# PatrykChrabaszcz/HpBandSter

Measured on AMD Instinct MI355X. Metric: candidate KDE evals/sec (cand×obs pairs) at D=32, 1/2/4/8 MI355X; % VALU peak, higher is better.
Workload: dtype f16 MFMA coarse pre-screen (1 product per dim, rigorous bound), f32 accumulate, f64 re-score

## Files before the change

hpbandster_amd/csrc/hbx_acq_impl.h:

```cpp
#pragma once
#include "hbx_kde_impl.h"
#include "hbx_score.h"

__device__ __forceinline__ void est_interval(const KdeEst e, float* lo, float* hi, float* pt) {
  const float m = fmaxf(e.lpos, e.lneg);
  if (m == -INFINITY) {
    *lo = *hi = *pt = -INFINITY;
    return;
  }
  const float a = __expf(e.lpos - m), b = __expf(e.lneg - m);
  const float S = a - b, E = e.err * (a + b) + 1e-6f * (a + b);
  *pt = S > 0.f ? m + __logf(S) : -INFINITY;
  *hi = (S + E) > 0.f ? m + __logf(S + E) + 1e-6f * fabsf(m) + 1e-5f : -INFINITY;
  *lo = (S - E) > 0.f ? m + __logf(S - E) - 1e-6f * fabsf(m) - 1e-5f : -INFINITY;
}

struct ScoreIv {
  float slo, shi, lpt, gpt;
  bool lnan, of, one;
};
__device__ __forceinline__ ScoreIv score_interval(const KdeEst a, const KdeEst b, const ScoreFloor F) {
  const float C = F.C;
  ScoreIv v;
  v.of = false;
// ... 30 lines not shown
}

#define HBX_EST_NOT_EVAL (-3.f)
__device__ __forceinline__ ScoreIv score_interval_l_only(const KdeEst a, const ScoreFloor F) {
  const float C = F.C;
  ScoreIv v;
  v.of = false;
  v.one = false;
  v.gpt = NAN;
  v.lnan = a.lpos != a.lpos;
  if (v.lnan) {
    v.slo = v.shi = NAN;
    v.lpt = NAN;
    return v;
  }
  float llo, lhi;
  est_interval(a, &llo, &lhi, &v.lpt);
  v.of = lhi > 700.f;
  v.slo = C - fmaxf(lhi, C) - F.w;
  v.shi = INFINITY;
  return v;
}

__device__ __forceinline__ KdeEst merge_splits(const KdeEst* __restrict__ e, int64_t stride, int64_t i, int nsplit) {
  KdeEst p[OBS_SPLIT_MAX];
#pragma unroll
  for (int r = 0; r < OBS_SPLIT_MAX; ++r) p[r] = r < nsplit ? e[(int64_t)r * stride + i] : kde_est_neutral();
  auto lae = [](float x, float y) {
    const float m = fmaxf(x, y);
    return m == -INFINITY ? m : m + __logf(__expf(x - m) + __expf(y - m));
  };
  KdeEst a = p[0];
#pragma unroll
  for (int r = 1; r < OBS_SPLIT_MAX; ++r) {
    if (r < nsplit) {
      const KdeEst b = p[r];
      if (a.lpos != a.lpos || b.lpos != b.lpos) {
        a.lpos = NAN;
      } else {
        a.lpos = lae(a.lpos, b.lpos);
        a.lneg = lae(a.lneg, b.lneg);
        const float ml = fmaxf(a.lpos > -INFINITY ? fabsf(a.lpos) : 0.f, a.lneg > -INFINITY ? fabsf(a.lneg) : 0.f);
        a.err = fmaxf(a.err, b.err) + 0x1p-18f + ml * 0x1p-22f;
      }
    }
  }
  return a;
}

__device__ __forceinline__ double bohb_score(double g, double l, double f) {
  return ((g > f) ? g : f) / ((f > l) ? f : l);
}

__device__ __forceinline__ double exact_rel(const KdeParams* __restrict__ P, const KdeEst e) {
  const double base = (8.0 * (double)P->D + 160.0) * 0x1p-52;
  if (!P->has_neg) return base;
  if (e.err < -1.5f) return INFINITY;
  const float m = fmaxf(e.lpos, e.lneg);
  if (!(m > -INFINITY)) return base;
  const float a = __expf(e.lpos - m), b = __expf(e.lneg - m);
  const float den = fabsf(a - b) - (e.err + 1e-6f) * (a + b);
  if (!(den > 0.f)) return INFINITY;
  return base * (double)((a + b) / den) * 1.01;
}

__device__ __forceinline__ double score_rel(const KdeParams* __restrict__ Pg, const KdeParams* __restrict__ Pb,
                                            const KdeEst* __restrict__ el, const KdeEst* __restrict__ eg,
                                            int64_t i) {
  return exact_rel(Pg, el[i]) + exact_rel(Pb, eg[i]) + 0x1p-51;
}
// ... 5 lines not shown
```

hpbandster_amd/csrc/hbx_acquire.h:

```cpp
#pragma once
#include "hbx_score.h"

struct KdePairRef {
  int32_t D;
  const void* params_good;
  const float* table_good;
  const double* X_good;
  const int64_t* rows_good;
  int32_t variant_good;
  const void* params_bad;
  const float* table_bad;
  const double* X_bad;
  const int64_t* rows_bad;
  int32_t variant_bad, dc_pad, du_pad;
  int64_t nmax;
  ScoreFloor floor;
  const KdeParams* Pg() const { return (const KdeParams*)params_good; }
  const KdeParams* Pb() const { return (const KdeParams*)params_bad; }
};

struct WsLayout {
  size_t res, U, count, flags, segcnt, segnear, best, key, first1, rescue, est_l, est_g, lo, list, near, exact_l,
      exact_g, part, total;
  size_t stage, seeds, surv, lpart, bmax;
// ... 55 lines not shown
int acq_check(const char* who, const KdePairRef& p, const double* cand, int64_t Nc, const void* workspace);
int acq_plan(const KdePairRef& p, bool fast, AcqPlan* plan);
int acq_score(const AcqPlan& plan, const KdePairRef& p, const AcqWs& a, const ScoreRequest& rq, int64_t batch_B,
              ScoreResult* out);
#ifndef HBX_STAGED_MIN_PAIRS
#define HBX_STAGED_MIN_PAIRS 1e9
#endif
#ifndef HBX_STAGED_TOPK_MIN_PAIRS
#define HBX_STAGED_TOPK_MIN_PAIRS 4e9
#endif
bool acq_staged_supported(const AcqPlan& plan);
int acq_score_staged(const AcqPlan& plan, const KdePairRef& p, const double* cand, int64_t Nc, const AcqWs& a,
                     hipEvent_t* ev, hipStream_t s, bool tail);
int staged_score_l(const AcqPlan& plan, const KdePairRef& p, const double* cand, int64_t Nc, const AcqWs& a,
                   hipEvent_t* ev, hipStream_t s, uint32_t* lkey, uint32_t* hist, int32_t hist_words,
                   unsigned* lhi_blocks = nullptr);
int staged_score_seeds(const AcqPlan& plan, const KdePairRef& p, const double* cand, int64_t Nc, const AcqWs& a,
                       hipStream_t s, bool mark_rest, bool update_u, unsigned lhi_blocks = 0);
int staged_score_survivors(const AcqPlan& plan, const KdePairRef& p, const double* cand, int64_t Nc, const AcqWs& a,
                           hipStream_t s, bool lonly);
int acq_exact_only_init(int64_t Nc, uint32_t seg, const AcqWs& a, hipStream_t s);
#define EXACT_SCAN_MAX 1024
int acq_exact(const KdePairRef& p, const double* cand, int64_t Nc, const AcqWs& a, bool scan, bool combine,
              hipStream_t s);
```

hpbandster_amd/csrc/hbx_common.h:

```cpp
#pragma once

#include <hip/hip_runtime.h>
#include <stdint.h>
#include <stdlib.h>

#define HBX_MAX_D 256
#define HBX_LO_TERMS 32
#define HBX_WAVE 64

#include "hbx.h"

int hbx_fail(int code, const char* fmt, ...);

#define HBX_HIP(call)                                                                 \
  do {                                                                                \
    hipError_t _e = (call);                                                           \
    if (_e != hipSuccess)                                                             \
      return hbx_fail(HBX_ERR_HIP, "%s failed: %s (%s:%d)", #call, hipGetErrorString(_e), \
                      __FILE__, __LINE__);                                            \
  } while (0)

#define HBX_LAUNCH_CHECK()                                                            \
  do {                                                                                \
    hipError_t _e = hipGetLastError();                                                \
// ... 15 lines not shown
static inline bool hbx_staged_tail() { return hbx_switch_on("HBX_STAGED_TAIL"); }
static inline bool hbx_stage1_lhi() { return hbx_switch_on("HBX_STAGE1_LHI"); }

struct KdeParams {
  int32_t n;
  int32_t D;
  int32_t dc;
  int32_t du;
  int32_t nconst;
  int32_t nan_all;
  int32_t has_neg;
  int32_t unsupported;
  int32_t stride;
  int32_t dc_pad;
  int32_t du_pad;
  int32_t exact_only;
  double log_norm;
  double m0_log2;
  double lb_sum;
  double prod_bw_c;
  float cmax;
  float sum_abs_delta;
  float cmax2;
  int32_t pad1;
  int32_t kc;
  int32_t hmode;
  int32_t nsc;
  int32_t chunk_floats;
  int32_t oh_total;
  int32_t coarse_off;
  int32_t coarse_chunk_floats;
  const double* X;
  const int64_t* rows;
  int32_t oh_dim[64];
  int32_t oh_level[64];
  int32_t oh_col[64];
  double oh_val[64];
  int32_t oh_start[64];
  int32_t cat_maxcode[HBX_MAX_D];
  int32_t cont_dim[HBX_MAX_D];
  double cont_scale[HBX_MAX_D];
  double center[HBX_MAX_D];
  float xmax[HBX_MAX_D];
  int32_t cat_dim[HBX_MAX_D];
  float cat_delta[HBX_MAX_D];
  float cat_negf[HBX_MAX_D];
  int32_t const_dim[HBX_MAX_D];
// ... 73 lines not shown
```

hpbandster_amd/csrc/hbx_exact.hip:

```cpp
#include "hbx_acquire.h"
#include "hbx_exact_impl.h"

#ifndef EXACT_ACQ_THREADS
#define EXACT_ACQ_THREADS 256
#endif
struct ExactScan {
  const float* lo;
  int64_t Nc;
  const uint32_t* U;
  const int32_t* flags;
  const int32_t* first1;
  int32_t* list;
  int32_t* count;
  int32_t* rescue_cnt;
};
template <bool SCAN>
__global__ __launch_bounds__(EXACT_ACQ_THREADS) void kde_exact_kernel(
    const double* __restrict__ cand, int32_t D,
    const KdeParams* __restrict__ Pg, const double* __restrict__ Xg, const int64_t* __restrict__ rows_g,
    const KdeParams* __restrict__ Pb, const double* __restrict__ Xb, const int64_t* __restrict__ rows_b,
    const int32_t* __restrict__ list_in, const int32_t* __restrict__ count, int32_t nbuf, double* __restrict__ part,
    double* __restrict__ exact_l, double* __restrict__ exact_g, ExactScan sc) {
  __shared__ ExactShared sh;
  __shared__ int32_t slist[SCAN ? EXACT_SCAN_MAX : 1];
  __shared__ int32_t swc[EXACT_ACQ_THREADS / 64];
  int cnt;
  const int32_t* list = list_in;
  if constexpr (SCAN) {
    const float u = hbx_ord2f(sc.U[0]);
    const bool all = (sc.flags[0] & 1) != 0;
    const int32_t f1 = sc.first1[0];
    const int lane = threadIdx.x & 63, wv = threadIdx.x >> 6;
    int base = 0;
    for (int64_t c0 = 0; c0 < sc.Nc; c0 += EXACT_ACQ_THREADS) {
      const int64_t i = c0 + threadIdx.x;
      bool in = false;
      if (i < sc.Nc) {
        const float l = sc.lo[i];
        in = (l == l && (all || l <= u)) || (int32_t)i == f1;
      }
      const uint64_t b = __ballot(in);
      if (lane == 0) swc[wv] = __popcll(b);
      __syncthreads();
      int off = base, tot = 0;
#pragma unroll
      for (int w = 0; w < EXACT_ACQ_THREADS / 64; ++w) {
        off += w < wv ? swc[w] : 0;
        tot += swc[w];
      }
      if (in) slist[off + __popcll(b & ((1ull << lane) - 1))] = (int32_t)i;
      base += tot;
      __syncthreads();
    }
    cnt = base;
    list = slist;
    if (blockIdx.x == 0) {
      for (int k = threadIdx.x; k < cnt; k += EXACT_ACQ_THREADS) sc.list[k] = slist[k];
      if (threadIdx.x == 0) {
        *sc.count = cnt;
        if (sc.rescue_cnt) *sc.rescue_cnt = 0;
      }
    }
  } else {
    cnt = *count;
  }
  const bool split = cnt <= EXACT_SPLIT_CAP;
  const int per = split ? nbuf * PW_SPLIT_UNITS : 1;
  const int64_t items = (int64_t)cnt * 2 * per;
  for (int64_t item = blockIdx.x; item < items; item += gridDim.x) {
    const int64_t pk = item / per;
    const int p = (int)(pk >> 1);
    const bool isl = pk & 1;
    const KdeParams* P = isl ? Pg : Pb;
    const double* X = isl ? Xg : Xb;
    const int64_t* rows = isl ? rows_g : rows_b;
    if (split) {
      const int r = (int)(item % per), b = r / PW_SPLIT_UNITS, u = r % PW_SPLIT_UNITS;
      const int n = P->n, c = b * PW_BUF;
      if (c >= n) continue;
      const int m = (n - c) < PW_BUF ? (n - c) : PW_BUF;
      int off, len;
      if (!pw_unit<PW_SPLIT_CUT>(m, u, &off, &len)) continue;
      exact_setup(P, D, cand + (int64_t)list[p] * D, &sh);
      const double v = exact_unit<PW_SPLIT_LEVELS>(X, D, rows, P, c + off, len, &sh);
      if (threadIdx.x == 0) part[pk * per + r] = v;
    } else {
      exact_setup(P, D, cand + (int64_t)list[p] * D, &sh);
      const double v = exact_pdf(X, D, rows, P, &sh);
      if (threadIdx.x == 0) (isl ? exact_l : exact_g)[p] = v;
    }
    __syncthreads();
  }
}

__global__ __launch_bounds__(256) void kde_exact_combine_kernel(const KdeParams* __restrict__ Pg,
                                                                const KdeParams* __restrict__ Pb,
                                                                const int32_t* __restrict__ count, int32_t nbuf,
                                                                const double* __restrict__ part,
                                                                double* __restrict__ exact_l,
                                                                double* __restrict__ exact_g) {
  const int cnt = *count;
  if (cnt > EXACT_SPLIT_CAP) return;
  const int64_t pk = (int64_t)blockIdx.x * 4 + (threadIdx.x >> 6);
  if (pk >= 2 * (int64_t)cnt) return;
  const bool isl = pk & 1;
  const int n = (isl ? Pg : Pb)->n;
  const double* us = part + pk * nbuf * PW_SPLIT_UNITS;
// ... 91 lines not shown
    if ((threadIdx.x & 63) == 0) {
      rm[threadIdx.x >> 6] = m;
      rs[threadIdx.x >> 6] = sm;
    }
    __syncthreads();
    if (threadIdx.x == 0) {
      double M = -INFINITY, Sx = 0.0;
      bool nan = false;
      for (int w = 0; w < 4; ++w) {
        if (rm[w] != rm[w]) nan = true;
        else if (rm[w] > -INFINITY) {
          const double mm = fmax(M, rm[w]);
          Sx = (M > -INFINITY ? Sx * exp(M - mm) : 0.0) + rs[w] * exp(rm[w] - mm);
          M = mm;
        }
      }
      out[p] = (nan || P->has_neg || P->nan_all || P->nconst) ? NAN : (M > -INFINITY ? M + log(Sx) + lconst : -INFINITY);
    }
    __syncthreads();
  }
}

int acq_exact(const KdePairRef& p, const double* cand, int64_t Nc, const AcqWs& a, bool scan, bool combine,
              hipStream_t s) {
  const int nbuf = (int)((p.nmax + PW_BUF - 1) / PW_BUF);
  const ExactScan esc = scan ? ExactScan{a.lo, Nc, a.U, a.flags, a.first1, a.list, a.count, a.rescue} : ExactScan{};
  auto ek = scan ? kde_exact_kernel<true> : kde_exact_kernel<false>;
  hipLaunchKernelGGL(ek, dim3(EXACT_GRID), dim3(EXACT_ACQ_THREADS), 0, s, cand, p.D, p.Pg(), p.X_good, p.rows_good,
                     p.Pb(), p.X_bad, p.rows_bad, a.list, a.count, nbuf, a.part, a.exact_l, a.exact_g, esc);
  HBX_LAUNCH_CHECK();
  if (combine) {
    hipLaunchKernelGGL(kde_exact_combine_kernel, dim3((2 * EXACT_SPLIT_CAP + 3) / 4), dim3(256), 0, s, p.Pg(), p.Pb(),
                       a.count, nbuf, a.part, a.exact_l, a.exact_g);
    HBX_LAUNCH_CHECK();
  }
  return HBX_OK;
}

int hbx_logpdf_exact_listed(const double* cand, int64_t Nc, int32_t D, const KdeParams* P, const double* X,
                            const int64_t* rows, double* out, const int32_t* list, const int32_t* count,
                            bool per_point, hipStream_t s) {
  const unsigned grid = (unsigned)(Nc < EXACT_GRID ? Nc : EXACT_GRID);
  if (per_point) {
    hipLaunchKernelGGL(kde_logpdf_exact_kernel, dim3(grid), dim3(256), 0, s, cand, Nc, D, P, X, rows, out, list, count);
    HBX_LAUNCH_CHECK();
  }
  hipLaunchKernelGGL(kde_pdf_exact_kernel, dim3(grid), dim3(EXACT_THREADS), 0, s, cand, Nc, D, P, X, rows, out, list,
                     count, 1);
  HBX_LAUNCH_CHECK();
  return HBX_OK;
}

// ... 45 lines not shown
```

hpbandster_amd/csrc/hbx_exact_impl.h:

```cpp
#pragma once
#include "hbx_kde_impl.h"
#include "hbx_npexp.h"
#include "hbx_pairwise.h"

struct ExactShared {
  double dens[PW_UNIT_MAX];
  double nsum[PW_LEVELS][128];
  double usum[PW_UNITS];
  double c0[HBX_MAX_D], c1[HBX_MAX_D], xd[HBX_MAX_D];
  int32_t cont[HBX_MAX_D];
};

template <typename PV>
__device__ void exact_setup(const PV* __restrict__ P, int32_t D, const double* __restrict__ x, ExactShared* sh) {
  for (int d = threadIdx.x; d < D; d += blockDim.x) {
    const double h = P->bw[d];
    const bool c = P->vartype[d] == 0;
    sh->cont[d] = c;
    sh->c0[d] = c ? (h * h) * 2. : 1. - h;
    sh->c1[d] = c ? 0. : h / (double)(P->nlev[d] - 1);
    sh->xd[d] = x[d];
  }
  __syncthreads();
}
// ... 3 lines not shown
                             const PV* __restrict__ P, int first, int len, ExactShared* sh) {
  const double pbc = P->prod_bw_c;
  for (int j = threadIdx.x; j < len; j += blockDim.x) {
    const double* xr = X + rows[first + j] * (int64_t)D;
    double p = 1.0;
#pragma unroll 8
    for (int d = 0; d < D; ++d) {
      const double v = xr[d], xv = sh->xd[d];
      double k;
      if (sh->cont[d]) {
        const double diff = v - xv;
        k = HBX_INV_SQRT_2PI * hbx_npexp::exp(-(diff * diff) / sh->c0[d]);
      } else {
        k = (v == xv) ? sh->c0[d] : sh->c1[d];
      }
      p = (d == 0) ? k : p * k;
    }
    sh->dens[j] = p / pbc;
  }
  __syncthreads();
  return np_pairwise_block<LEVELS>(sh->dens, len, sh->nsum);
}

template <typename PV>
__device__ double exact_pdf(const double* __restrict__ X, int32_t D, const int64_t* __restrict__ rows,
                            const PV* __restrict__ P, ExactShared* sh) {
  const int n = P->n;
  double acc = 0.0;
  for (int c = 0; c < n; c += PW_BUF) {
    const int m = (n - c) < PW_BUF ? (n - c) : PW_BUF;
    for (int u = 0; u < PW_UNITS; ++u) {
      int off, len;
      if (!pw_unit(m, u, &off, &len)) continue;
      const double v = exact_unit(X, D, rows, P, c + off, len, sh);
      if (threadIdx.x == 0) sh->usum[u] = v;
    }
    __syncthreads();
    if (threadIdx.x == 0) acc = acc + pw_combine_units(m, sh->usum);
  }
  return acc / (double)n;
}
```

hpbandster_amd/csrc/hbx_kde.hip:

```cpp
#include "hbx_acquire.h"

#include <string.h>

#include <new>

#include "hbx_acq_impl.h"
#include "hbx_host.h"
#include "hbx_pairwise.h"
#include "hbx_rescue_impl.h"


__global__ void acq_init_kernel(uint32_t* U, int32_t* count, int32_t* flags, int32_t* first1, AcqResult* res) {
  if (threadIdx.x == 0 && blockIdx.x == 0) acq_init_state(U, count, flags, first1, res);
}

__global__ void acq_init_batch_kernel(int64_t B, uint32_t* __restrict__ U, int32_t* __restrict__ flags,
                                      int32_t* __restrict__ segcnt, uint64_t* __restrict__ best,
                                      uint64_t* __restrict__ key, int32_t* __restrict__ first1,
                                      int32_t* __restrict__ count, int32_t* __restrict__ segnear) {
  const int64_t b = (int64_t)blockIdx.x * blockDim.x + threadIdx.x;
  if (b == 0) *count = 0;
  if (b < B) {
    U[b] = hbx_f2ord(INFINITY);
    flags[b] = 0;
// ... 580 lines not shown
  const dim3 grid((unsigned)((Nc + 255) / 256));
  bool fuse_combine = false;
  if (Nc > 0) {
    if (plan.exact_only) {
      rc = acq_exact_only_init(Nc, sg, a, s);
      if (rc) return rc;
    } else if (!tail) {
      const CombineRescue rs{cand, p.D, p.Pg(), p.Pb(), a.rescue};
      const bool sgn = KdeVariant::decode(p.variant_good).has_neg;
      const combine_fn cf = !rescue_inline ? kde_combine_kernel<false, false>
                            : sgn          ? kde_combine_kernel<true, true>
                                           : kde_combine_kernel<false, true>;
      hipLaunchKernelGGL(cf, dim3((unsigned)((Nc + 256 * COMBINE_SUB - 1) / (256 * COMBINE_SUB))), dim3(256), 0, s,
                         a.el, a.eg, Nc, sg, logl_out, logg_out, a.lo, a.U, a.flags, a.first1, rs, p.floor);
      HBX_LAUNCH_CHECK();
    }
    const bool scan = !batch_res && Nc <= EXACT_SCAN_MAX && !tail;
    if (!scan && !tail) {
      hipLaunchKernelGGL(kde_shortlist_kernel, grid, dim3(256), 0, s, a.lo, Nc, sg, a.U, a.flags, a.list, a.count,
                         batch_res ? a.segcnt : (int32_t*)nullptr, a.first1, a.rescue);
      HBX_LAUNCH_CHECK();
    }
    fuse_combine = !batch_res && !(plan.exact_only && (logl_out || logg_out));
    rc = acq_exact(p, cand, Nc, a, scan, !fuse_combine, s);
    if (rc) return rc;
    if (plan.exact_only && (logl_out || logg_out)) {
      hipLaunchKernelGGL(kde_exact_logs_kernel, grid, dim3(256), 0, s, a.list, a.count, a.exact_l, a.exact_g, logl_out,
                         logg_out);
      HBX_LAUNCH_CHECK();
    }
  }
  if (!batch_res) {
    hipLaunchKernelGGL(kde_final_kernel, dim3(1), dim3(256), 0, s, a.list, a.count, a.exact_l, a.exact_g, a.flags,
                       c.index_base, p.Pg(), p.Pb(), a.el, a.eg, a.near, a.res,
                       (int32_t)((p.nmax + PW_BUF - 1) / PW_BUF), fuse_combine ? a.part : (const double*)nullptr,
                       a.exact_l, a.exact_g, c.host_res, c.seq, c.pick, p.floor.f);
    HBX_LAUNCH_CHECK();
    return HBX_OK;
  }
  if (Nc > 0) {
    hipLaunchKernelGGL(kde_batch_min_kernel, grid, dim3(256), 0, s, a.list, a.count, sg, a.exact_l, a.exact_g, a.best,
                       p.floor.f);
    HBX_LAUNCH_CHECK();
    hipLaunchKernelGGL(kde_batch_key_kernel, grid, dim3(256), 0, s, a.list, a.count, sg, a.exact_l, a.exact_g, a.best,
                       a.key, p.floor.f);
    HBX_LAUNCH_CHECK();
    hipLaunchKernelGGL(kde_batch_near_kernel, grid, dim3(256), 0, s, a.list, a.count, sg, a.exact_l, a.exact_g, a.key,
// ... 113 lines not shown
```

hpbandster_amd/csrc/hbx_prep.hip:

```cpp
#include <math.h>
#include <string.h>

#include "hbx_prep.h"
#include "hbx_sort.h"

__host__ __device__ static int table_stride(int dc_pad, int du_pad) { return chunk_floats(dc_pad, du_pad); }
static int64_t n_chunks(int64_t n) { return (n + OBS_CHUNK - 1) / OBS_CHUNK; }
__device__ __forceinline__ int64_t n_chunks_dev(int64_t n) { return (n + OBS_CHUNK - 1) / OBS_CHUNK; }
static int64_t table_floats(int64_t n, int dc_pad, int du_pad) {
  if (dc_pad < 0 || du_pad < 0) return 1;
  int a = chunk_floats(dc_pad, du_pad, 0, 0), b = chunk_floats(dc_pad, du_pad, OH_MAX_KC, 1);
  const int c = h_chunk_floats(dc_pad, OH_MAX_KC, 1), d = h32_chunk_floats(nsc_of(dc_pad), OH_MAX_KC, 1);
  a = a > b ? a : b;
  a = a > d ? a : d;
  const int e = h32c_chunk_floats(nsc_of(dc_pad), 2);
  return n_chunks(n) * (int64_t)((a > c ? a : c) + e);
}

__device__ __forceinline__ void prep_publish_rows(const PrepPub& q, int k, int t, int nt) {
  const uint64_t tag = (uint64_t)(uint32_t)q.seq << 32;
  auto put = [&](int64_t i, uint32_t w) {
    __hip_atomic_store(q.dst + i, tag | w, __ATOMIC_RELAXED, __HIP_MEMORY_SCOPE_SYSTEM);
  };
  if (k == 0) {
// ... 172 lines not shown
      sad += (kd == 1 && 1.0 - h != 0.0) ? fabsf((float)(la - lb)) : 0.f;
      one_pos = one_pos || (kd == 2 && h > 0.0);
    }
    int dcp, dup;
    bucket_dims(S.dc_tot, S.du_tot, &dcp, &dup);
    P->n = n;
    P->D = D;
    P->dc_pad = dcp;
    P->du_pad = dup;
    const int exo = (dcp < 0 || dup < 0 || one_pos) ? 1 : 0;
    P->exact_only = exo;
    P->stride = (dcp < 0 || dup < 0) ? 0 : table_stride(dcp, dup);
    const int dc = S.dc_tot;
    P->dc = dc;
    P->du = S.du;
    S.dcp = dcp;
    S.dup = dup;
    S.exo = exo;
    P->nconst = S.nconst;
    P->m0_log2 = m0;
    P->lb_sum = lb_sum;
    P->prod_bw_c = prod_bw_c;
    P->sum_abs_delta = sad;
    P->log_norm = -log((double)n) - sum_ln_h - 0.5 * (double)dc * log(2.0 * M_PI) + m0 * M_LN2;
    P->X = A.X;
    P->rows = A.rows;
  }
  __syncthreads();
  if (blockIdx.x == 0) PSTAMP(2);
  for (int t = tid; t < 64; t += blockDim.x) {
    P->oh_col[t] = 0;
    P->oh_val[t] = NAN;
  }
  const int du = S.du;
  if (tid == 0) {
    int tot = 0;
    bool ok = true;
    for (int u = 0; u < du; ++u) {
      if (S.cm[u] < 0) {
        ok = false;
      } else {
        S.ohs[u] = (tot + 1) & ~1;
        tot = S.ohs[u] + S.cm[u] + 1;
      }
    }
    S.kc = (!S.exo && du > 0 && ok && 2 * tot <= 32 * OH_MAX_KC && tot <= 64) ? (2 * tot + 31) / 32 : 0;
    S.tot = tot;
// ... 576 lines not shown
```

hpbandster_amd/csrc/hbx_score_h32.hip:

```cpp
#include "hbx_common.h"
#include "hbx_kde_impl.h"
#include "hbx_acq_impl.h"
#include "hbx_pick.h"

typedef float f32x16 __attribute__((ext_vector_type(16)));
typedef uint32_t u32x2 __attribute__((ext_vector_type(2)));
typedef uint32_t u32x4 __attribute__((ext_vector_type(4)));

#define H32_CMAX 30000.f

constexpr int h32_waves(bool co) { return co ? H32C_WAVES : H16_WAVES; }
constexpr int h32_cands(bool co, int ct) { return 32 * ct * h32_waves(co); }

template <int KS> struct H32Idx { typedef u32x4 T; };
template <> struct H32Idx<1> { typedef u32x2 T; };
template <> struct H32Idx<2> { typedef u32x2 T; };
template <int KS, typename T> __device__ __forceinline__ int h32_idx(const T& v, int s, int h) {
  if constexpr (KS == 1) return (int)(h ? v[1] : v[0]);
  else return (int)v[s];
}

template <int I, int NM, int NV, int NRL, bool RD = true>
struct SgbH32 {
  static __device__ __forceinline__ void run() {
    __builtin_amdgcn_sched_group_barrier(0x008, 1, 0);
    constexpr int nr = !RD ? 0 : I == NM - 1 ? NRL : 1;
    if constexpr (nr > 0) __builtin_amdgcn_sched_group_barrier(0x100, nr, 0);
    constexpr int n = NV / NM + (I < NV % NM ? 1 : 0);
    if constexpr (n > 0) __builtin_amdgcn_sched_group_barrier(0x002, n, 0);
    SgbH32<I + 1, NM, NV, NRL, RD>::run();
  }
};
template <int NM, int NV, int NRL, bool RD>
struct SgbH32<NM, NM, NV, NRL, RD> {
  static __device__ __forceinline__ void run() {}
};

__device__ __forceinline__ void stage_rows_list(const double* __restrict__ cand, const int32_t* __restrict__ idx,
                                                int64_t nv, int D, int DS, double* xs, int lane) {
  const int tot = (int)nv * D;
  for (int e0 = 0; e0 < tot; e0 += 8 * 64) {
    double t[8];
// ... 273 lines not shown
#pragma unroll
    for (int s = 0; s < KL; ++s) {
      acc = __builtin_amdgcn_smfmac_f32_32x32x32_f16(asl[s], bsp[t][s], acc, h32_idx<KS>(aix, s, h), 0, 0);
      asl[s] = *(const f16x8*)(a + 16 * ND + 16 * KP + 16 * s);
      if (!SG && s == KL - 1) aix = *(const typename H32Idx<KS>::T*)(a + ixo);
    }
    if constexpr (SG) {
#pragma unroll
      for (int s = 0; s < KS; ++s) {
        accp = __builtin_amdgcn_smfmac_f32_32x32x32_f16(apar[s], bsp[t][s], s == 0 ? zero16 : accp, h32_idx<KS>(aix, s, h),
                                                        0, 0);
        apar[s] = *(const f16x8*)(a + PAR + 16 * s);
        if (s == KS - 1) aix = *(const typename H32Idx<KS>::T*)(a + ixo);
      }
    }
  };
#pragma unroll
  for (int t = 0; t < CT; ++t) {
    f32x16 a0, a1;
    readA(lds, 0);
    mma(a0, t);
    readA(lds, 1);
    mma(a1, t);
    float mx = fmaxf(a0[0], a1[0]);
#pragma unroll
    for (int r = 1; r < 16; ++r) mx = fmaxf(mx, fmaxf(a0[r], a1[r]));
    mx = fmaxf(mx, __shfl_xor(mx, 32));
    const float d = rintf(-(ci[t] + mx));
    const float dl = (d > 0.f && d < 1e30f) ? d : 0.f;
    const float cs = ci[t] + dl;
    const bool big = fabsf(cs) > H32_CMAX;
    const float cv = big ? 0.f : cs;
    const _Float16 p0 = (_Float16)cv;
    const float r1 = cv - (float)p0;
    const _Float16 p1 = (_Float16)r1;
    const _Float16 p2 = (_Float16)(r1 - (float)p1);
    if (h == 0) {
      bd[t][0][3] = p0;
      bd[t][0][4] = p1;
      bd[t][0][5] = p2;
    }
    if (h == 0) {
      float* ax = aux + ((wave * CT + t) * 32 + c) * 4;
      ax[0] = ci[t];
      ax[1] = bnd[t];
      ax[2] = dl;
      ax[3] = big ? -1.f : cer[t] * (1.f + 0x1p-18f);
    }
  }
// ... 337 lines not shown
```

hpbandster_amd/csrc/hbx_staged.hip:

```cpp
#include "hbx_acquire.h"

#include <hip/hip_ext.h>

#include "hbx_acq_impl.h"
#include "hbx_rescue_impl.h"

#define STAGED_PT 4
#define HBX_LN4f 1.3862943611198906f
#define STAGED_SEED_BLOCKS 2048

template <bool KEYS>
__global__ __launch_bounds__(256) void staged_l_kernel(KdeEst* __restrict__ el, int64_t Nc, int32_t ns,
                                                       const double* __restrict__ cand, int32_t D,
                                                       const KdeParams* __restrict__ Pl,
                                                       const int32_t* __restrict__ rescue_cnt,
                                                       float* __restrict__ lhi, uint32_t* __restrict__ stage,
                                                       uint32_t* __restrict__ lkey, uint32_t* __restrict__ hist,
                                                       int32_t hist_words) {
  if constexpr (KEYS) {
    if (blockIdx.x == 0)
      for (int j = threadIdx.x; j < hist_words; j += 256) hist[j] = 0;
  }
  const int32_t nres = *rescue_cnt;
  KdeEst e[STAGED_PT];
// ... 51 lines not shown
  if (lane == 63) wtot[wv] = incl;
  __syncthreads();
  int woff = 0, total = 0;
  for (int w = 0; w < 4; ++w) {
    if (w < wv) woff += wtot[w];
    total += wtot[w];
  }
  if (threadIdx.x == 0) base = total > 0 ? atomicAdd(count, total) : 0;
  __syncthreads();
  return base + woff + incl - n;
}

__global__ __launch_bounds__(256) void staged_seed_kernel(float* __restrict__ lhi, int64_t Nc,
                                                          KdeEst* __restrict__ eg, int32_t* __restrict__ seeds,
                                                          int32_t cap, uint32_t* __restrict__ stage,
                                                          int32_t mark_rest, const float* __restrict__ bmax,
                                                          int32_t nblk, const double* __restrict__ cand, int32_t D,
                                                          const KdeParams* __restrict__ Pl,
                                                          KdeEst* __restrict__ el) {
  float lmax;
  if (bmax) {
    __shared__ float rb[4];
    float m = -INFINITY;
    for (int j = threadIdx.x; j < nblk; j += 256) m = fmaxf(m, bmax[j]);
    for (int o = 32; o > 0; o >>= 1) m = fmaxf(m, __shfl_xor(m, o));
    if ((threadIdx.x & 63) == 0) rb[threadIdx.x >> 6] = m;
    __syncthreads();
    lmax = fmaxf(fmaxf(rb[0], rb[1]), fmaxf(rb[2], rb[3]));
    if (blockIdx.x == 0 && threadIdx.x == 0) {
      stage[HBX_ST_LMAX] = hbx_f2ord(lmax);
      stage[HBX_ST_LHI1] = 1;
    }
  } else {
    lmax = hbx_ord2f(stage[HBX_ST_LMAX]);
  }
  const float thr = lmax - HBX_LN4f;
  const int64_t ntile = (Nc + 256 * STAGED_PT - 1) / (256 * STAGED_PT);
  for (int64_t tb = blockIdx.x; tb < ntile; tb += gridDim.x) {
  bool f[STAGED_PT];
  int n = 0;
#pragma unroll
  for (int r = 0; r < STAGED_PT; ++r) {
    const int64_t i = (tb * STAGED_PT + r) * 256 + threadIdx.x;
    f[r] = false;
    if (i < Nc) {
      float h = lhi[i];
      if (bmax && h == INFINITY) {
// ... 25 lines not shown
      }
      ++off;
    }
    if (seeded) lhi[i] = NAN;
    else if (mark_rest) eg[i] = none;
  }
  }
}

__global__ __launch_bounds__(256) void staged_merge_kernel(const KdeEst* __restrict__ part, int32_t cap, int32_t ns,
                                                           const int32_t* __restrict__ idx,
                                                           const int32_t* __restrict__ count, int32_t maxcount,
                                                           const KdeEst* __restrict__ el, KdeEst* __restrict__ eg,
                                                           const KdeParams* __restrict__ Pb,
                                                           uint32_t* __restrict__ stage, int32_t update_u,
                                                           ScoreFloor F) {
  int32_t cnt = *count;
  if (cnt > maxcount) cnt = maxcount;
  if (cnt > cap) return;
  const int32_t k = blockIdx.x * 256 + threadIdx.x;
  float h = INFINITY;
  if (k < cnt) {
    const int32_t i = idx[k];
    bool mark = false;
    for (int q = 0; q < ns; ++q) mark = mark || part[(int64_t)q * cap + k].err == -1.f;
    KdeEst e = {0.f, -INFINITY, -1.f, 0.f};
    if (!mark) e = merge_splits(part, cap, k, ns);
    eg[i] = e;
    if (update_u && !mark) {
      const ScoreIv v = score_interval(el[i], e, F);
      if (!v.lnan) h = v.shi;
    }
  }
  if (update_u) {
    const bool guard = Pb->log_norm + log((double)(Pb->n > 1 ? Pb->n : 1)) < 600.0;
    for (int o = 32; o > 0; o >>= 1) h = fminf(h, __shfl_xor(h, o));
    if ((threadIdx.x & 63) == 0 && guard && h < INFINITY) {
      const uint32_t o = hbx_f2ord(h);
      if (o < __hip_atomic_load(stage + HBX_ST_USEED, __ATOMIC_RELAXED, __HIP_MEMORY_SCOPE_AGENT))
        atomicMin(stage + HBX_ST_USEED, o);
    }
  }
}

__global__ __launch_bounds__(256) void staged_survivor_kernel(float* __restrict__ lhi, int64_t Nc,
                                                              int32_t* __restrict__ surv,
                                                              uint32_t* __restrict__ stage,
                                                              int32_t* __restrict__ flags, ScoreFloor F) {
  const float U = hbx_ord2f(stage[HBX_ST_USEED]);
  const float C = F.C;
  bool f[STAGED_PT];
  int n = 0;
#pragma unroll
  for (int r = 0; r < STAGED_PT; ++r) {
    const int64_t i = ((int64_t)blockIdx.x * STAGED_PT + r) * 256 + threadIdx.x;
    f[r] = false;
    if (i < Nc) {
      const float h = lhi[i];
// ... 68 lines not shown
    const int64_t k = (int64_t)blockIdx.x * EPB + r * TAIL_THREADS_A + threadIdx.x;
    idx[r] = -1;
    if (k < total) idx[r] = k < nseed ? t.seeds[k] : t.surv[k - nseed];
  }
#pragma unroll
  for (int r = 0; r < TAIL_PT; ++r) {
    const int64_t k = (int64_t)blockIdx.x * EPB + r * TAIL_THREADS_A + threadIdx.x;
    if (idx[r] < 0) continue;
    ea[r] = t.el[idx[r]];
    if (k < nseed || !split) eb[r] = t.eg[idx[r]];
  }
  float h = INFINITY;
  int32_t f1 = INT32_MAX;
  bool of = false;
#pragma unroll
  for (int r = 0; r < TAIL_PT; ++r) {
    const int64_t k = (int64_t)blockIdx.x * EPB + r * TAIL_THREADS_A + threadIdx.x;
    slo[r] = NAN;
    if (idx[r] < 0) continue;
    const int64_t i = idx[r];
    bool store = false;
    if (!(k < nseed || !split)) {
      const int64_t ks = k - nseed;
      bool mark = false;
      for (int q = 0; q < t.ns; ++q) mark = mark || t.part[(int64_t)q * t.cap + ks].err == -1.f;
      eb[r] = {0.f, -INFINITY, -1.f, 0.f};
      if (!mark) eb[r] = merge_splits(t.part, t.cap, ks, t.ns);
      store = true;
    }
    if (nres != 0 && eb[r].err == -1.f) {
      eb[r] = kde_rescue_one<0, false, true>(t.cand, i, t.D, t.Pb);
      store = true;
    }
    if (store) t.eg[i] = eb[r];
    const ScoreIv v = score_interval(ea[r], eb[r], t.F);
    slo[r] = v.one ? NAN : v.slo;
    t.lo[i] = slo[r];
    if (!v.lnan) h = fminf(h, v.shi);
    if (v.one && (int32_t)i < f1) f1 = (int32_t)i;
    of = of || v.of;
  }
  float hw = h;
  int32_t fw = f1;
  for (int o = 32; o > 0; o >>= 1) {
    hw = fminf(hw, __shfl_xor(hw, o));
    fw = min(fw, __shfl_xor(fw, o));
  }
  const bool ofw = __ballot(of) != 0;
  bool lowered = false;
  if (lane == 0) {
// ... 236 lines not shown
```

hpbandster_amd/csrc/hbx_topk.hip:

```cpp
#include "hbx_acq_impl.h"
#include "hbx_acquire.h"
#include "hbx_rescue_impl.h"
#include "hbx_topk_rank.h"

#define TOPK_KEY_INF 0xFF800000u
#define TOPK_HIST_WORDS (4 * 256)

__global__ __launch_bounds__(256) void topk_bounds_kernel(const KdeEst* __restrict__ el,
                                                          const KdeEst* __restrict__ eg, int64_t Nc,
                                                          float* __restrict__ lo, uint32_t* __restrict__ hik,
                                                          int32_t* __restrict__ flags, uint32_t* __restrict__ hist,
                                                          ScoreFloor F) {
  if (blockIdx.x == 0)
    for (int j = threadIdx.x; j < TOPK_HIST_WORDS; j += 256) hist[j] = 0;
  const int64_t i = (int64_t)blockIdx.x * 256 + threadIdx.x;
  bool of = false;
  if (i < Nc) {
    const ScoreIv v = score_interval(el[i], eg[i], F);
    of = v.of;
    const float l = v.lnan ? NAN : (v.slo == v.slo ? v.slo : -INFINITY);
    const float h = (v.lnan || v.shi != v.shi) ? INFINITY : v.shi;
    lo[i] = l;
    hik[i] = hbx_f2ord(h);
  }
// ... 169 lines not shown
      for (int q = 0; q < 4; ++q) {
        c[q] = hb[4 * t + q];
        sum += c[q];
      }
      uint32_t incl = sum;
      for (int o = 1; o < 64; o <<= 1) {
        const uint32_t v = __shfl_up(incl, o);
        if (t >= o) incl += v;
      }
      uint32_t run = incl - sum;
#pragma unroll
      for (int q = 0; q < 4; ++q) {
        if (run < rank && rank <= run + c[q]) {
          s_prefix = prefix | ((uint32_t)(4 * t + q) << shift);
          s_rank = rank - run;
        }
        run += c[q];
      }
      if (t == 63 && incl < rank) s_rank = 0xffffffffu;
    }
    __syncthreads();
  }
  if (t == 0) {
    const bool guard = Pb->log_norm + log((double)(Pb->n > 1 ? Pb->n : 1)) < 600.0;
    stage[HBX_ST_USEED] = guard && s_rank != 0xffffffffu ? s_prefix : TOPK_KEY_INF;
  }
}

struct TopkStagedArgs {
  const KdeEst* part;
  int32_t cap, ns;
  TopkEval ev;
  int64_t Nc;
  const double* cand;
  int32_t D;
  const KdeParams* Pb;
  const KdeEst* el;
  KdeEst* eg;
  float* lo;
  uint32_t* ekey;
  int32_t* flags;
  const int32_t* rescue_cnt;
  ScoreFloor F;
};
__global__ __launch_bounds__(256) void topk_staged_bounds_kernel(TopkStagedArgs t) {
  int64_t nseed = (int32_t)t.ev.stage[HBX_ST_NSEED], nsurv = (int32_t)t.ev.stage[HBX_ST_NSURV];
  if (nseed > t.cap) nseed = t.cap;
// ... 236 lines not shown
```

Baseline: 31360 billion.

## Spread exact re-score across lanes, fuse split merge loads, and micro-optimise reductions

Adds a wide exact re-score kernel that assigns each observation to a group of 4 lanes, splits the dimensions across them and combines the per-dimension kernel products with shuffles; it is used on the tail path. Split merging now loads each partial once and checks the marker in the same pass, instead of reading the partials twice. The h32 max reduction uses v_max3 with two accumulators, the bmax reduction reads float4, and the log-pdf guard is computed once at prep time instead of calling log() in kernels. The wide kernel launches 1024-thread blocks, which may reduce occupancy, and its shuffle products add work per dimension.

```diff
diff --git a/hpbandster_amd/csrc/hbx_acq_impl.h b/hpbandster_amd/csrc/hbx_acq_impl.h
--- a/hpbandster_amd/csrc/hbx_acq_impl.h
+++ b/hpbandster_amd/csrc/hbx_acq_impl.h
@@ -76,10 +76,7 @@
   return v;
 }
 
-__device__ __forceinline__ KdeEst merge_splits(const KdeEst* __restrict__ e, int64_t stride, int64_t i, int nsplit) {
-  KdeEst p[OBS_SPLIT_MAX];
-#pragma unroll
-  for (int r = 0; r < OBS_SPLIT_MAX; ++r) p[r] = r < nsplit ? e[(int64_t)r * stride + i] : kde_est_neutral();
+__device__ __forceinline__ KdeEst merge_loaded_splits(const KdeEst (&p)[OBS_SPLIT_MAX], int nsplit) {
   auto lae = [](float x, float y) {
     const float m = fmaxf(x, y);
     return m == -INFINITY ? m : m + __logf(__expf(x - m) + __expf(y - m));
@@ -100,6 +97,27 @@
     }
   }
   return a;
+}
+__device__ __forceinline__ void load_splits(KdeEst (&p)[OBS_SPLIT_MAX], const KdeEst* __restrict__ e, int64_t stride,
+                                            int64_t i, int nsplit) {
+#pragma unroll
+  for (int r = 0; r < OBS_SPLIT_MAX; ++r) p[r] = r < nsplit ? e[(int64_t)r * stride + i] : kde_est_neutral();
+}
+__device__ __forceinline__ KdeEst merge_splits(const KdeEst* __restrict__ e, int64_t stride, int64_t i, int nsplit) {
+  KdeEst p[OBS_SPLIT_MAX];
+  load_splits(p, e, stride, i, nsplit);
+  return merge_loaded_splits(p, nsplit);
+}
+__device__ __forceinline__ KdeEst merge_splits_or_marker(const KdeEst* __restrict__ e, int64_t stride, int64_t i,
+                                                         int nsplit, bool* mark) {
+  KdeEst p[OBS_SPLIT_MAX];
+  load_splits(p, e, stride, i, nsplit);
+  bool m = false;
+#pragma unroll
+  for (int r = 0; r < OBS_SPLIT_MAX; ++r) m = m || (r < nsplit && p[r].err == -1.f);
+  *mark = m;
+  const KdeEst a = merge_loaded_splits(p, nsplit);
+  return m ? KdeEst{0.f, -INFINITY, -1.f, 0.f} : a;
 }
 
 __device__ __forceinline__ double bohb_score(double g, double l, double f) {
diff --git a/hpbandster_amd/csrc/hbx_acquire.h b/hpbandster_amd/csrc/hbx_acquire.h
--- a/hpbandster_amd/csrc/hbx_acquire.h
+++ b/hpbandster_amd/csrc/hbx_acquire.h
@@ -101,4 +101,4 @@
 int acq_exact_only_init(int64_t Nc, uint32_t seg, const AcqWs& a, hipStream_t s);
 #define EXACT_SCAN_MAX 1024
 int acq_exact(const KdePairRef& p, const double* cand, int64_t Nc, const AcqWs& a, bool scan, bool combine,
-              hipStream_t s);
+              hipStream_t s, bool wide = false);
diff --git a/hpbandster_amd/csrc/hbx_common.h b/hpbandster_amd/csrc/hbx_common.h
--- a/hpbandster_amd/csrc/hbx_common.h
+++ b/hpbandster_amd/csrc/hbx_common.h
@@ -61,7 +61,7 @@
   float cmax;
   float sum_abs_delta;
   float cmax2;
-  int32_t pad1;
+  int32_t lnpdf_guard;
   int32_t kc;
   int32_t hmode;
   int32_t nsc;
diff --git a/hpbandster_amd/csrc/hbx_exact.hip b/hpbandster_amd/csrc/hbx_exact.hip
--- a/hpbandster_amd/csrc/hbx_exact.hip
+++ b/hpbandster_amd/csrc/hbx_exact.hip
@@ -1,9 +1,8 @@
 #include "hbx_acquire.h"
 #include "hbx_exact_impl.h"
 
-#ifndef EXACT_ACQ_THREADS
 #define EXACT_ACQ_THREADS 256
-#endif
+#define EXACT_ACQ_LANES 4
 struct ExactScan {
   const float* lo;
   int64_t Nc;
@@ -14,8 +13,8 @@
   int32_t* count;
   int32_t* rescue_cnt;
 };
-template <bool SCAN>
-__global__ __launch_bounds__(EXACT_ACQ_THREADS) void kde_exact_kernel(
+template <bool SCAN, int LANES>
+__global__ __launch_bounds__(EXACT_ACQ_THREADS * LANES) void kde_exact_kernel(
     const double* __restrict__ cand, int32_t D,
     const KdeParams* __restrict__ Pg, const double* __restrict__ Xg, const int64_t* __restrict__ rows_g,
     const KdeParams* __restrict__ Pb, const double* __restrict__ Xb, const int64_t* __restrict__ rows_b,
@@ -23,7 +22,8 @@
     double* __restrict__ exact_l, double* __restrict__ exact_g, ExactScan sc) {
   __shared__ ExactShared sh;
   __shared__ int32_t slist[SCAN ? EXACT_SCAN_MAX : 1];
-  __shared__ int32_t swc[EXACT_ACQ_THREADS / 64];
+  constexpr int NT = EXACT_ACQ_THREADS * LANES;
+  __shared__ int32_t swc[NT / 64];
   int cnt;
   const int32_t* list = list_in;
   if constexpr (SCAN) {
@@ -32,7 +32,7 @@
     const int32_t f1 = sc.first1[0];
     const int lane = threadIdx.x & 63, wv = threadIdx.x >> 6;
     int base = 0;
-    for (int64_t c0 = 0; c0 < sc.Nc; c0 += EXACT_ACQ_THREADS) {
+    for (int64_t c0 = 0; c0 < sc.Nc; c0 += NT) {
       const int64_t i = c0 + threadIdx.x;
       bool in = false;
       if (i < sc.Nc) {
@@ -44,7 +44,7 @@
       __syncthreads();
       int off = base, tot = 0;
 #pragma unroll
-      for (int w = 0; w < EXACT_ACQ_THREADS / 64; ++w) {
+      for (int w = 0; w < NT / 64; ++w) {
         off += w < wv ? swc[w] : 0;
         tot += swc[w];
       }
@@ -55,7 +55,7 @@
     cnt = base;
     list = slist;
     if (blockIdx.x == 0) {
-      for (int k = threadIdx.x; k < cnt; k += EXACT_ACQ_THREADS) sc.list[k] = slist[k];
+      for (int k = threadIdx.x; k < cnt; k += NT) sc.list[k] = slist[k];
       if (threadIdx.x == 0) {
         *sc.count = cnt;
         if (sc.rescue_cnt) *sc.rescue_cnt = 0;
@@ -82,7 +82,9 @@
       int off, len;
       if (!pw_unit<PW_SPLIT_CUT>(m, u, &off, &len)) continue;
       exact_setup(P, D, cand + (int64_t)list[p] * D, &sh);
-      const double v = exact_unit<PW_SPLIT_LEVELS>(X, D, rows, P, c + off, len, &sh);
+      double v;
+      if constexpr (LANES > 1) v = exact_unit_spread<PW_SPLIT_LEVELS, LANES>(X, D, rows, P, c + off, len, &sh);
+      else v = exact_unit<PW_SPLIT_LEVELS>(X, D, rows, P, c + off, len, &sh);
       if (threadIdx.x == 0) part[pk * per + r] = v;
     } else {
       exact_setup(P, D, cand + (int64_t)list[p] * D, &sh);
@@ -220,12 +222,16 @@
 }
 
 int acq_exact(const KdePairRef& p, const double* cand, int64_t Nc, const AcqWs& a, bool scan, bool combine,
-              hipStream_t s) {
+              hipStream_t s, bool wide) {
+  if (scan && wide) return hbx_fail(HBX_ERR_ARG, "acq_exact: the wide re-score does not scan");
   const int nbuf = (int)((p.nmax + PW_BUF - 1) / PW_BUF);
   const ExactScan esc = scan ? ExactScan{a.lo, Nc, a.U, a.flags, a.first1, a.list, a.count, a.rescue} : ExactScan{};
-  auto ek = scan ? kde_exact_kernel<true> : kde_exact_kernel<false>;
-  hipLaunchKernelGGL(ek, dim3(EXACT_GRID), dim3(EXACT_ACQ_THREADS), 0, s, cand, p.D, p.Pg(), p.X_good, p.rows_good,
-                     p.Pb(), p.X_bad, p.rows_bad, a.list, a.count, nbuf, a.part, a.exact_l, a.exact_g, esc);
+  auto ek = wide   ? kde_exact_kernel<false, EXACT_ACQ_LANES>
+            : scan ? kde_exact_kernel<true, 1>
+                   : kde_exact_kernel<false, 1>;
+  const dim3 threads(EXACT_ACQ_THREADS * (wide ? EXACT_ACQ_LANES : 1));
+  hipLaunchKernelGGL(ek, dim3(EXACT_GRID), threads, 0, s, cand, p.D, p.Pg(), p.X_good, p.rows_good, p.Pb(), p.X_bad,
+                     p.rows_bad, a.list, a.count, nbuf, a.part, a.exact_l, a.exact_g, esc);
   HBX_LAUNCH_CHECK();
   if (combine) {
     hipLaunchKernelGGL(kde_exact_combine_kernel, dim3((2 * EXACT_SPLIT_CAP + 3) / 4), dim3(256), 0, s, p.Pg(), p.Pb(),
diff --git a/hpbandster_amd/csrc/hbx_exact_impl.h b/hpbandster_amd/csrc/hbx_exact_impl.h
--- a/hpbandster_amd/csrc/hbx_exact_impl.h
+++ b/hpbandster_amd/csrc/hbx_exact_impl.h
@@ -49,6 +49,59 @@
   return np_pairwise_block<LEVELS>(sh->dens, len, sh->nsum);
 }
 
+#define EXACT_SPREAD_ROUNDS 2
+template <int LEVELS, int T, typename PV>
+__device__ double exact_unit_spread(const double* __restrict__ X, int32_t D, const int64_t* __restrict__ rows,
+                                    const PV* __restrict__ P, int first, int len, ExactShared* sh) {
+  static_assert(T >= 1 && T <= 64 && (T & (T - 1)) == 0, "a group lies within one wave");
+  const double pbc = P->prod_bw_c;
+  const int t = threadIdx.x & (T - 1), nobs = blockDim.x / T;
+  for (int j0 = 0; j0 < len; j0 += nobs) {
+    const int j = j0 + (int)threadIdx.x / T;
+    const bool act = j < len;
+    const double* xr = X + rows[first + (act ? j : 0)] * (int64_t)D;
+    double p = 1.0;
+    double vn[EXACT_SPREAD_ROUNDS];
+#pragma unroll
+    for (int q = 0; q < EXACT_SPREAD_ROUNDS; ++q) vn[q] = xr[q * T + t < D ? q * T + t : D - 1];
+    for (int d0 = 0; d0 < D; d0 += T * EXACT_SPREAD_ROUNDS) {
+      double v[EXACT_SPREAD_ROUNDS], k[EXACT_SPREAD_ROUNDS];
+#pragma unroll
+      for (int q = 0; q < EXACT_SPREAD_ROUNDS; ++q) {
+        const int dn = d0 + (EXACT_SPREAD_ROUNDS + q) * T + t;
+        v[q] = vn[q];
+        vn[q] = xr[dn < D ? dn : D - 1];
+      }
+#pragma unroll
+      for (int q = 0; q < EXACT_SPREAD_ROUNDS; ++q) {
+        const int d = d0 + q * T + t < D ? d0 + q * T + t : D - 1;
+        k[q] = 1.0;
+        if (d0 + q * T < D) {
+          const double xv = sh->xd[d];
+          if (sh->cont[d]) {
+            const double diff = v[q] - xv;
+            k[q] = HBX_INV_SQRT_2PI * hbx_npexp::exp(-(diff * diff) / sh->c0[d]);
+          } else {
+            k[q] = (v[q] == xv) ? sh->c0[d] : sh->c1[d];
+          }
+        }
+      }
+#pragma unroll
+      for (int q = 0; q < EXACT_SPREAD_ROUNDS; ++q) {
+#pragma unroll
+        for (int s = 0; s < T; ++s) {
+          const double ks = __shfl(k[q], s, T);
+          const int d = d0 + q * T + s;
+          if (d < D) p = (d == 0) ? ks : p * ks;
+        }
+      }
+    }
+    if (act && t == 0) sh->dens[j] = p / pbc;
+  }
+  __syncthreads();
+  return np_pairwise_block<LEVELS>(sh->dens, len, sh->nsum);
+}
+
 template <typename PV>
 __device__ double exact_pdf(const double* __restrict__ X, int32_t D, const int64_t* __restrict__ rows,
                             const PV* __restrict__ P, ExactShared* sh) {
diff --git a/hpbandster_amd/csrc/hbx_kde.hip b/hpbandster_amd/csrc/hbx_kde.hip
--- a/hpbandster_amd/csrc/hbx_kde.hip
+++ b/hpbandster_amd/csrc/hbx_kde.hip
@@ -626,7 +626,7 @@
       HBX_LAUNCH_CHECK();
     }
     fuse_combine = !batch_res && !(plan.exact_only && (logl_out || logg_out));
-    rc = acq_exact(p, cand, Nc, a, scan, !fuse_combine, s);
+    rc = acq_exact(p, cand, Nc, a, scan, !fuse_combine, s, tail);
     if (rc) return rc;
     if (plan.exact_only && (logl_out || logg_out)) {
       hipLaunchKernelGGL(kde_exact_logs_kernel, grid, dim3(256), 0, s, a.list, a.count, a.exact_l, a.exact_g, logl_out,
diff --git a/hpbandster_amd/csrc/hbx_prep.hip b/hpbandster_amd/csrc/hbx_prep.hip
--- a/hpbandster_amd/csrc/hbx_prep.hip
+++ b/hpbandster_amd/csrc/hbx_prep.hip
@@ -218,7 +218,9 @@
     P->lb_sum = lb_sum;
     P->prod_bw_c = prod_bw_c;
     P->sum_abs_delta = sad;
-    P->log_norm = -log((double)n) - sum_ln_h - 0.5 * (double)dc * log(2.0 * M_PI) + m0 * M_LN2;
+    const double log_norm = -log((double)n) - sum_ln_h - 0.5 * (double)dc * log(2.0 * M_PI) + m0 * M_LN2;
+    P->log_norm = log_norm;
+    P->lnpdf_guard = log_norm + log((double)(n > 1 ? n : 1)) < 600.0 ? 1 : 0;
     P->X = A.X;
     P->rows = A.rows;
   }
diff --git a/hpbandster_amd/csrc/hbx_score_h32.hip b/hpbandster_amd/csrc/hbx_score_h32.hip
--- a/hpbandster_amd/csrc/hbx_score_h32.hip
+++ b/hpbandster_amd/csrc/hbx_score_h32.hip
@@ -18,6 +18,12 @@
 template <int KS, typename T> __device__ __forceinline__ int h32_idx(const T& v, int s, int h) {
   if constexpr (KS == 1) return (int)(h ? v[1] : v[0]);
   else return (int)v[s];
+}
+
+__device__ __forceinline__ float h32_max3(float a, float b, float c) {
+  float r;
+  asm("v_max3_f32 %0, %1, %2, %3" : "=v"(r) : "v"(a), "v"(b), "v"(c));
+  return r;
 }
 
 template <int I, int NM, int NV, int NRL, bool RD = true>
@@ -337,9 +343,13 @@
     mma(a0, t);
     readA(lds, 1);
     mma(a1, t);
-    float mx = fmaxf(a0[0], a1[0]);
-#pragma unroll
-    for (int r = 1; r < 16; ++r) mx = fmaxf(mx, fmaxf(a0[r], a1[r]));
+    float mx = fmaxf(a0[0], a1[0]), my = fmaxf(a0[1], a1[1]);
+#pragma unroll
+    for (int r = 2; r < 16; r += 2) {
+      mx = h32_max3(mx, a0[r], a1[r]);
+      my = h32_max3(my, a0[r + 1], a1[r + 1]);
+    }
+    mx = fmaxf(mx, my);
     mx = fmaxf(mx, __shfl_xor(mx, 32));
     const float d = rintf(-(ci[t] + mx));
     const float dl = (d > 0.f && d < 1e30f) ? d : 0.f;
diff --git a/hpbandster_amd/csrc/hbx_staged.hip b/hpbandster_amd/csrc/hbx_staged.hip
--- a/hpbandster_amd/csrc/hbx_staged.hip
+++ b/hpbandster_amd/csrc/hbx_staged.hip
@@ -97,7 +97,17 @@
   if (bmax) {
     __shared__ float rb[4];
     float m = -INFINITY;
-    for (int j = threadIdx.x; j < nblk; j += 256) m = fmaxf(m, bmax[j]);
+    const float4* b4 = (const float4*)bmax;
+    const int n4 = nblk >> 2;
+    for (int j = threadIdx.x; j < n4; j += 4 * 256) {
+      float4 v[4];
+#pragma unroll
+      for (int q = 0; q < 4; ++q)
+        v[q] = j + q * 256 < n4 ? b4[j + q * 256] : make_float4(-INFINITY, -INFINITY, -INFINITY, -INFINITY);
+#pragma unroll
+      for (int q = 0; q < 4; ++q) m = fmaxf(m, fmaxf(fmaxf(v[q].x, v[q].y), fmaxf(v[q].z, v[q].w)));
+    }
+    for (int j = (n4 << 2) + threadIdx.x; j < nblk; j += 256) m = fmaxf(m, bmax[j]);
     for (int o = 32; o > 0; o >>= 1) m = fmaxf(m, __shfl_xor(m, o));
     if ((threadIdx.x & 63) == 0) rb[threadIdx.x >> 6] = m;
     __syncthreads();
@@ -169,18 +179,17 @@
   float h = INFINITY;
   if (k < cnt) {
     const int32_t i = idx[k];
-    bool mark = false;
-    for (int q = 0; q < ns; ++q) mark = mark || part[(int64_t)q * cap + k].err == -1.f;
-    KdeEst e = {0.f, -INFINITY, -1.f, 0.f};
-    if (!mark) e = merge_splits(part, cap, k, ns);
+    const KdeEst a = update_u ? el[i] : kde_est_neutral();
+    bool mark;
+    const KdeEst e = merge_splits_or_marker(part, cap, k, ns, &mark);
     eg[i] = e;
     if (update_u && !mark) {
-      const ScoreIv v = score_interval(el[i], e, F);
+      const ScoreIv v = score_interval(a, e, F);
       if (!v.lnan) h = v.shi;
     }
   }
   if (update_u) {
-    const bool guard = Pb->log_norm + log((double)(Pb->n > 1 ? Pb->n : 1)) < 600.0;
+    const bool guard = Pb->lnpdf_guard != 0;
     for (int o = 32; o > 0; o >>= 1) h = fminf(h, __shfl_xor(h, o));
     if ((threadIdx.x & 63) == 0 && guard && h < INFINITY) {
       const uint32_t o = hbx_f2ord(h);
@@ -295,10 +304,8 @@
     bool store = false;
     if (!(k < nseed || !split)) {
       const int64_t ks = k - nseed;
-      bool mark = false;
-      for (int q = 0; q < t.ns; ++q) mark = mark || t.part[(int64_t)q * t.cap + ks].err == -1.f;
-      eb[r] = {0.f, -INFINITY, -1.f, 0.f};
-      if (!mark) eb[r] = merge_splits(t.part, t.cap, ks, t.ns);
+      bool mark;
+      eb[r] = merge_splits_or_marker(t.part, t.cap, ks, t.ns, &mark);
       store = true;
     }
     if (nres != 0 && eb[r].err == -1.f) {
diff --git a/hpbandster_amd/csrc/hbx_topk.hip b/hpbandster_amd/csrc/hbx_topk.hip
--- a/hpbandster_amd/csrc/hbx_topk.hip
+++ b/hpbandster_amd/csrc/hbx_topk.hip
@@ -215,7 +215,7 @@
     __syncthreads();
   }
   if (t == 0) {
-    const bool guard = Pb->log_norm + log((double)(Pb->n > 1 ? Pb->n : 1)) < 600.0;
+    const bool guard = Pb->lnpdf_guard != 0;
     stage[HBX_ST_USEED] = guard && s_rank != 0xffffffffu ? s_prefix : TOPK_KEY_INF;
   }
 }
```

New measurement: 32310 billion, median of 6. 3.1% higher.
